# lukifer23/Matrix0

Measured on AMD Instinct MI355X. Metric: self-play games/sec at 800 sims/move, ResNet-24 53M; 1/2/4/8 MI355X, higher is better.
Workload: dtype f16

## Files before the change

matrix0_amd/csrc/attn_block.hip:

```cpp
#include "kernel_common.h"
#include "conv_epilogue.h"

typedef _Float16 half4v __attribute__((ext_vector_type(4)));
typedef float float4v __attribute__((ext_vector_type(4)));

namespace {
constexpr int AB_PIECE = 12288;
constexpr int AB_PIECES_PER_GROUP = 7;
constexpr int AB_GROUPS = 10;
constexpr int AB_X = 0;
constexpr int AB_QK = 81920;
constexpr int AB_VT = AB_QK + 16384;
constexpr int AB_VROW = 68;
constexpr int AB_RING = AB_VT + 4 * 16 * AB_VROW * 2;
constexpr int AB_PAR = AB_RING + 4 * AB_PIECE;
constexpr int AB_LDS = AB_PAR + 4 * 320 * 4;
}

__device__ __forceinline__ void ab_load64(half8& b0, half8& b1, half8& b2, half8& b3, const half8* p) {
    asm volatile("global_load_dwordx4 %0, %4, off\n\tglobal_load_dwordx4 %1, %4, off offset:16\n\t"
                 "global_load_dwordx4 %2, %4, off offset:32\n\tglobal_load_dwordx4 %3, %4, off offset:48"
                 : "=&v"(b0), "=&v"(b1), "=&v"(b2), "=&v"(b3) : "v"(p) : "memory");
}
template <int OFF>
__device__ __forceinline__ void ab_lds16(half8& d, uint32_t addr) {
    asm volatile("ds_read_b128 %0, %1 offset:%2" : "=v"(d) : "v"(addr), "n"(OFF) : "memory");
}
template <int N>
__device__ __forceinline__ void ab_lds_arrived(half8& f0, half8& f1, half8& f2, half8& f3, half8& f4, half8& f5) {
    static_assert(N == 0 || N == 5, "");
    if constexpr (N == 0) asm volatile("s_waitcnt lgkmcnt(0)" : "+v"(f0), "+v"(f1), "+v"(f2), "+v"(f3), "+v"(f4), "+v"(f5) :: "memory");
    else asm volatile("s_waitcnt lgkmcnt(5)" : "+v"(f0), "+v"(f1), "+v"(f2), "+v"(f3), "+v"(f4), "+v"(f5) :: "memory");
}
template <int CTRL>
__device__ __forceinline__ float ab_dpp(float v) {
    return __builtin_bit_cast(float, __builtin_amdgcn_update_dpp(0, __builtin_bit_cast(int, v), CTRL, 0xF, 0xF, true));
}
__device__ __forceinline__ float ab_row_sum(float v) {
    v += ab_dpp<0xB1>(v);
    v += ab_dpp<0x4E>(v);
    v += ab_dpp<0x141>(v);
    v += ab_dpp<0x140>(v);
    return v;
}

#ifndef AB_DBG
#define AB_DBG 0
#endif
#define AB_WAIT(n) asm volatile("s_waitcnt vmcnt(" #n ")" ::: "memory")
#if defined(AB_STAMP) || defined(AB_STAMP2) || defined(AB_STAMP3)
__device__ unsigned long long* g_ab_stamp;
#ifdef AB_STAMP
#define AB_ST(k) do { if (tid == 0) g_ab_stamp[(size_t)blockIdx.x * 16 + (k)] = __builtin_amdgcn_s_memtime(); } while (0)
#else
#define AB_ST(k) do {} while (0)
#endif
#else
#define AB_ST(k) do {} while (0)
#endif
#define AB_LGKM0() asm volatile("s_waitcnt lgkmcnt(0)" ::: "memory")
#ifdef AB_STAMP3
#define AB_T3(k) do { if (g == 5) ts[k] = __builtin_amdgcn_s_memtime(); } while (0)
#else
#define AB_T3(k) do {} while (0)
#endif
#ifdef AB_STAMP2
#define AB_TS(k) do { if (g == 5) ts[k] = __builtin_amdgcn_s_memtime(); } while (0)
#else
#define AB_TS(k) do {} while (0)
#endif

template <int ACT>
__global__ __launch_bounds__(512) void attn_block_kernel(AttnBlockArgs a) {
    extern __shared__ __attribute__((aligned(16))) char smem[];
    const int tid = threadIdx.x, lane = tid & 63;
    const int w = __builtin_amdgcn_readfirstlane(tid >> 6);
    const int l15 = lane & 15, lq = lane >> 4, r31 = lane & 31, half = lane >> 5;
    const int wm = w >> 1, wn = w & 1;
    const size_t b0 = (size_t)blockIdx.x * 2;
    const char* xg = reinterpret_cast<const char*>(a.x) + b0 * 64 * 640;

    AB_ST(0);
#pragma unroll
    for (int n = 0; n < 10; ++n) {
        const int idx = w * 10 + n;
        const int q = idx * 64 + lane;
        const int row = q / 40, pos = q - row * 40;
        const int src = (pos & ~7) | ((pos ^ (row >> 1)) & 7);
        glds16(xg + row * 640 + src * 16, smem + AB_X + idx * 1024);
    }
    const char* wsrc = reinterpret_cast<const char*>(a.wpack) + w * 1536 + lane * 16;
    char* const ring_w = smem + AB_RING + w * 1536;
    auto issue = [&](int t) __attribute__((always_inline)) {
        const char* s = wsrc + (size_t)t * AB_PIECE;
        char* d = ring_w + (t & 3) * AB_PIECE;
        glds16(s, d);
        if (lane < 32) glds16(s + 1024, d + 1024);
    };
    issue(0); issue(1); issue(2);
    if (tid < 320) {
        float* par = reinterpret_cast<float*>(smem + AB_PAR);
        par[tid] = a.ln_g[tid]; par[320 + tid] = a.ln_b[tid];
        par[640 + tid] = a.y2 ? a.gn2_gamma[tid] : 0.f; par[960 + tid] = a.y2 ? a.gn2_beta[tid] : 0.f;
    }

#if AB_DBG == 3
    AB_WAIT(0);
    __syncthreads();
    if (blockIdx.x == 0)
        for (int i = tid; i < 3 * AB_PIECE / 4; i += 512)
            reinterpret_cast<uint32_t*>(a.y)[i] = reinterpret_cast<const uint32_t*>(smem + AB_RING)[i];
    return;
#endif
    const int au = w >> 1, aboard = au >> 1, ahl = au & 1, aqt = w & 1;
    const int aq = aqt * 32 + r31;
    half2v visp[16];
    {
        const uint64_t m = a.mask[aq];
        static_for<0, 32>([&](auto i_) __attribute__((always_inline)) {
            constexpr int i = decltype(i_)::value;
            constexpr int kt = i >> 4, r = i & 15;
            const int key = kt * 32 + 8 * (r >> 2) + 4 * half + (r & 3);
            visp[i >> 1][i & 1] = (_Float16)(float)((m >> key) & 1);
        });
    }
    float wm_, wu_;
    if (a.mix > 0.f && a.mix < 1.f) { wm_ = 1.f - a.mix; wu_ = 1.f - (1.f - a.mix); }
    else if (a.mix >= 1.f) { wm_ = 1.f; wu_ = 0.f; }
    else { wm_ = 0.f; wu_ = 1.f; }
    const float isd = a.inv_sqrt_d * 1.44269504088896f;
    const float clampv = 50.f * 1.44269504088896f;

    const int xrow0 = 32 * wm + l15;
    const int xsw = (xrow0 >> 1) & 7;
    const int xe0 = ((lq ^ xsw) & 7) * 16, xe1 = (((4 + lq) ^ xsw) & 7) * 16;
    const uint32_t lds0 = (uint32_t)(uintptr_t)smem;
    const uint32_t xa[2] = {lds0 + AB_X + xrow0 * 640 + xe0, lds0 + AB_X + xrow0 * 640 + xe1};
    const int wsw = (l15 >> 1) & 7;
    const int wq0 = (3 * wn * 16 + l15) * 128 + ((lq ^ wsw) & 7) * 16;
    const int wq1 = (3 * wn * 16 + l15) * 128 + (((4 + lq) ^ wsw) & 7) * 16;
    const int wpo = l15 * 64 + ((lq ^ (4 - (l15 >> 2))) & 3) * 16;
    const uint32_t ring_a = lds0 + AB_RING;
    const uint32_t of_a = lds0 + AB_QK + (lq >> 1) * 4096 + (16 * w + l15) * 32 + ((lq & 1) ^ (l15 >> 3)) * 16;

    const float4v zero4 = {0.f, 0.f, 0.f, 0.f};
    const float16v zero16 = {0.f, 0.f, 0.f, 0.f, 0.f, 0.f, 0.f, 0.f, 0.f, 0.f, 0.f, 0.f, 0.f, 0.f, 0.f, 0.f};
    float4v oc[20];
    static_for<0, 20>([&](auto j_) __attribute__((always_inline)) { oc[decltype(j_)::value] = zero4; });

#if defined(AB_STAMP2) || defined(AB_STAMP3)
    unsigned long long ts[10] = {0, 0, 0, 0, 0, 0, 0, 0, 0, 0};
#endif
    half8 fs[2][5];
    half8 of;
    float4v qa[2][3];
    half8 bias8[4];
    auto sequence = [&](auto hp_, auto hq_, const int T, const int g) __attribute__((always_inline)) {
        constexpr bool HP = decltype(hp_)::value, HQ = decltype(hq_)::value;
        constexpr int NP = (HP ? 2 : 0) + (HQ ? 5 : 0), NU = 2 * NP;
        constexpr int BU = NU - 3;
        auto load = [&](auto u_) __attribute__((always_inline)) {
            constexpr int u = decltype(u_)::value, S = u & 1, i = u >> 1, kk = u & 1;
            const uint32_t slot = ring_a + (uint32_t)(((T + i) & 3) * AB_PIECE);
            if constexpr (HP && i < 2) {
                if constexpr (u == 0) ab_lds16<0>(of, of_a);
                const uint32_t pa = slot + wpo;
                static_for<0, 5>([&](auto jj_) __attribute__((always_inline)) {
                    constexpr int jj = decltype(jj_)::value;
                    ab_lds16<(5 * kk + jj) * 1024>(fs[S][jj], pa);
                });
            } else {
                constexpr int p = i - (HP ? 2 : 0);
                ab_lds16<128 * p>(fs[S][3], xa[kk]);
                ab_lds16<128 * p + 16 * 640>(fs[S][4], xa[kk]);
                const uint32_t wa = slot + (kk ? wq1 : wq0);
                static_for<0, 3>([&](auto j_) __attribute__((always_inline)) {
                    constexpr int j = decltype(j_)::value;
                    ab_lds16<j * 2048>(fs[S][j], wa);
                });
            }
        };
        auto arrived = [&](auto u_, auto n_) __attribute__((always_inline)) {
            constexpr int S = decltype(u_)::value & 1;
            ab_lds_arrived<decltype(n_)::value>(fs[S][0], fs[S][1], fs[S][2], fs[S][3], fs[S][4], of);
        };
        auto mma = [&](auto u_) __attribute__((always_inline)) {
            constexpr int u = decltype(u_)::value, S = u & 1, i = u >> 1, kk = u & 1;
            if constexpr (HP && i < 2) {
                static_for<0, 5>([&](auto jj_) __attribute__((always_inline)) {
                    constexpr int c = 10 * i + 5 * kk + decltype(jj_)::value;
                    oc[c] = __builtin_amdgcn_mfma_f32_16x16x32_f16(fs[S][decltype(jj_)::value], of, oc[c], 0, 0, 0);
                });
            } else {
                static_for<0, 3>([&](auto j_) __attribute__((always_inline)) {
                    constexpr int j = decltype(j_)::value;
                    qa[0][j] = __builtin_amdgcn_mfma_f32_16x16x32_f16(fs[S][j], fs[S][3], qa[0][j], 0, 0, 0);
                    qa[1][j] = __builtin_amdgcn_mfma_f32_16x16x32_f16(fs[S][j], fs[S][4], qa[1][j], 0, 0, 0);
                });
            }
        };
        if constexpr (HP && HQ) AB_TS(0);
        AB_LGKM0();
        AB_WAIT(4);
        __builtin_amdgcn_s_barrier();
        asm volatile("" ::: "memory");
        if constexpr (HP && HQ) AB_TS(1);
        load(std::integral_constant<int, 0>{});
        issue(T + 3);
        static_for<0, NU>([&](auto u_) __attribute__((always_inline)) {
            constexpr int u = decltype(u_)::value;
            if constexpr (u + 1 < NU) {
                if constexpr (u & 1) {
                    if constexpr (HP && HQ && u == 7) AB_T3(7);
                    arrived(u_, std::integral_constant<int, 0>{});
                    if constexpr (HP && HQ && u == 7) AB_T3(8);
                    AB_WAIT(4);
                    __builtin_amdgcn_s_barrier();
                    asm volatile("" ::: "memory");
                    if constexpr (HP && HQ && u == 5) AB_T3(0);
                    if constexpr (HP && HQ && u == 7) AB_T3(9);
                    if constexpr (HP && HQ && (u == 1 || u == 3 || u == 7 || u == 11)) { if (g == 5) AB_ST(u == 1 ? 12 : u == 3 ? 13 : u == 7 ? 14 : 15); }
                    if constexpr (HP && HQ) AB_TS(2 + (u >> 1));
                }
                load(std::integral_constant<int, u + 1>{});
                if constexpr (HP && HQ && u == 5) AB_T3(1);
                if constexpr (HP && HQ && u == 6) AB_T3(4);
                if constexpr (u & 1) issue(T + (u >> 1) + 4);
                else arrived(u_, std::integral_constant<int, 5>{});
                if constexpr (HP && HQ && u == 5) AB_T3(2);
                if constexpr (HP && HQ && u == 6) AB_T3(5);
            } else {
                arrived(u_, std::integral_constant<int, 0>{});
            }
            if constexpr (HQ && u == BU) {
                const half8* bp = reinterpret_cast<const half8*>(a.bias) + ((size_t)((2 * g + ahl) * 2 + aqt) * 64 + lane) * 4;
                ab_load64(bias8[0], bias8[1], bias8[2], bias8[3], bp);
            }
            mma(u_);
            __builtin_amdgcn_sched_barrier(0);
            if constexpr (HP && HQ && u == 5) AB_T3(3);
            if constexpr (HP && HQ && u == 6) AB_T3(6);
            if constexpr (HP && HQ && u == NU - 1) AB_TS(8);
        });
    };

    auto zero_qa = [&]() __attribute__((always_inline)) {
        static_for<0, 2>([&](auto i_) __attribute__((always_inline)) {
            static_for<0, 3>([&](auto j_) __attribute__((always_inline)) { qa[decltype(i_)::value][decltype(j_)::value] = zero4; });
        });
    };
    auto stage_and_attend = [&](const int g) __attribute__((always_inline)) {
        if (g == 5) AB_ST(5);
        static_for<0, 2>([&](auto i_) __attribute__((always_inline)) {
            static_for<0, 3>([&](auto j_) __attribute__((always_inline)) {
                constexpr int i = decltype(i_)::value, j = decltype(j_)::value;
                const int J = 3 * wn + j, type = J >> 1, hl = J & 1;
                const int token = 32 * wm + 16 * i + l15;
                const half4v h = {(_Float16)qa[i][j][0], (_Float16)qa[i][j][1], (_Float16)qa[i][j][2], (_Float16)qa[i][j][3]};
                if (type < 2) {
                    *reinterpret_cast<half4v*>(smem + AB_QK + type * 8192 + hl * 4096 + token * 32 + (((lq >> 1) ^ (l15 >> 3)) & 1) * 16 + (lq & 1) * 8) = h;
                } else {
                    const int unit = (token >> 6) * 2 + hl, sq = token & 63;
                    union { half2v h2; uint32_t u; } p01, p23;
                    p01.h2 = half2v{h[0], h[1]}; p23.h2 = half2v{h[2], h[3]};
                    const bool odd = (lane & 1) != 0;
                    const uint32_t own = odd ? p23.u : p01.u;
                    const uint32_t recv = (uint32_t)__builtin_amdgcn_update_dpp(0, (int)(odd ? p01.u : p23.u), 0xB1, 0xF, 0xF, true);
                    const uint32_t ta = odd ? recv : own, tb = odd ? own : recv;
                    const uint32_t w0 = __builtin_amdgcn_perm(tb, ta, 0x05040100u);
                    const uint32_t w1 = __builtin_amdgcn_perm(tb, ta, 0x07060302u);
                    uint32_t* vt = reinterpret_cast<uint32_t*>(reinterpret_cast<_Float16*>(smem + AB_VT) +
                                                               (unit * 16 + 4 * lq + (odd ? 2 : 0)) * AB_VROW + (sq & ~1));
                    vt[0] = w0; vt[AB_VROW / 2] = w1;
                }
            });
        });
        AB_LGKM0();
        __builtin_amdgcn_s_barrier();
        asm volatile("" ::: "memory");
        if (g == 5) AB_ST(6);
        AB_TS(9);
        if (AB_DBG != 2) {
            const char* Kb = smem + AB_QK + 8192 + ahl * 4096 + aboard * 64 * 32;
            const int hsw = 16 * (half ^ ((r31 >> 3) & 1));
            const half8 kf0 = *reinterpret_cast<const half8*>(Kb + r31 * 32 + hsw);
            const half8 kf1 = *reinterpret_cast<const half8*>(Kb + (32 + r31) * 32 + hsw);
            char* Qp = smem + AB_QK + ahl * 4096 + (aboard * 64 + aq) * 32 + hsw;
            const half8 qfr = *reinterpret_cast<const half8*>(Qp);
            half8 vf[2][2];
            {
                const _Float16* vrow = reinterpret_cast<const _Float16*>(smem + AB_VT) + (au * 16 + l15) * AB_VROW;
                static_for<0, 2>([&](auto kt_) __attribute__((always_inline)) {
                    static_for<0, 2>([&](auto jb_) __attribute__((always_inline)) {
                        constexpr int kt = decltype(kt_)::value, jb = decltype(jb_)::value;
                        const half4v lo = *reinterpret_cast<const half4v*>(vrow + kt * 32 + 16 * jb + 4 * half);
                        const half4v hi = *reinterpret_cast<const half4v*>(vrow + kt * 32 + 16 * jb + 8 + 4 * half);
                        vf[kt][jb] = half8{lo[0], lo[1], lo[2], lo[3], hi[0], hi[1], hi[2], hi[3]};
                    });
                });
            }
            float16v st[2];
            st[0] = __builtin_amdgcn_mfma_f32_32x32x16_f16(kf0, qfr, zero16, 0, 0, 0);
            st[1] = __builtin_amdgcn_mfma_f32_32x32x16_f16(kf1, qfr, zero16, 0, 0, 0);
            asm volatile("s_waitcnt vmcnt(0)" : "+v"(bias8[0]), "+v"(bias8[1]), "+v"(bias8[2]), "+v"(bias8[3]) :: "memory");
            float e[2][16];
            float su = 0.f, sm = 0.f;
            static_for<0, 2>([&](auto kt_) __attribute__((always_inline)) {
                static_for<0, 16>([&](auto r_) __attribute__((always_inline)) {
                    constexpr int kt = decltype(kt_)::value, r = decltype(r_)::value;
                    constexpr int bi = kt * 16 + r;
                    float d = st[kt][r] * isd + (float)bias8[bi >> 3][bi & 7];
                    d = __builtin_amdgcn_fmed3f(d, -clampv, clampv);
                    const float eu = __builtin_amdgcn_exp2f(d);
                    e[kt][r] = eu;
                    su += eu;
                    sm += eu * (float)visp[bi >> 1][bi & 1];
                });
            });
            su += __shfl_xor(su, 32);
            sm += __shfl_xor(sm, 32);
            const float cu = wu_ / su, cm = wm_ / sm;
            float16v oacc = zero16;
            static_for<0, 2>([&](auto kt_) __attribute__((always_inline)) {
                static_for<0, 2>([&](auto jb_) __attribute__((always_inline)) {
                    constexpr int kt = decltype(kt_)::value, jb = decltype(jb_)::value;
                    half8 pf;
                    static_for<0, 8>([&](auto u_) __attribute__((always_inline)) {
                        constexpr int u = decltype(u_)::value;
                        constexpr int r = 8 * jb + u, bi = kt * 16 + r;
                        const float vis = (float)visp[bi >> 1][bi & 1];
                        pf[u] = (_Float16)(e[kt][r] * (vis * cm + cu));
                    });
                    oacc = __builtin_amdgcn_mfma_f32_32x32x16_f16(vf[kt][jb], pf, oacc, 0, 0, 0);
                });
            });
            union { half2v h2[2]; uint32_t u[2]; } lo4, hi4, rcv;
            lo4.h2[0] = half2v{(_Float16)oacc[0], (_Float16)oacc[1]}; lo4.h2[1] = half2v{(_Float16)oacc[2], (_Float16)oacc[3]};
            hi4.h2[0] = half2v{(_Float16)oacc[4], (_Float16)oacc[5]}; hi4.h2[1] = half2v{(_Float16)oacc[6], (_Float16)oacc[7]};
            rcv.u[0] = __shfl_xor(half ? lo4.u[0] : hi4.u[0], 32);
            rcv.u[1] = __shfl_xor(half ? lo4.u[1] : hi4.u[1], 32);
            typedef uint32_t uint4v __attribute__((ext_vector_type(4)));
            uint4v ov;
            if (half == 0) ov = uint4v{lo4.u[0], lo4.u[1], rcv.u[0], rcv.u[1]};
            else ov = uint4v{rcv.u[0], rcv.u[1], hi4.u[0], hi4.u[1]};
            asm volatile("ds_write_b128 %0, %1" :: "v"((uint32_t)(uintptr_t)Qp), "v"(ov) : "memory");
        }
        if (g == 5) AB_ST(7);
    };

    if (AB_DBG != 1) {
        zero_qa();
        sequence(std::false_type{}, std::true_type{}, 0, 0);
#pragma unroll 1
        for (int g = 0; g < AB_GROUPS - 1; ++g) {
            stage_and_attend(g);
            if (g == 4) AB_ST(8);
            if (g == 5) AB_ST(11);
            zero_qa();
            sequence(std::true_type{}, std::true_type{}, 7 * g + 5, g + 1);
        }
        stage_and_attend(AB_GROUPS - 1);
        sequence(std::true_type{}, std::false_type{}, 7 * AB_GROUPS - 2, AB_GROUPS);
    }
    AB_ST(2);
#if defined(AB_STAMP2) || defined(AB_STAMP3)
    if (lane == 0 && (w & 3) == 0)
        for (int k = 0; k < 10; ++k) g_ab_stamp[((size_t)blockIdx.x * 2 + (w >> 2)) * 16 + k] = ts[k];
#endif
    AB_WAIT(0);
    __syncthreads();

    const int token = 16 * w + l15;
    const int tsw = (token >> 1) & 7;
    char* xrow = smem + AB_X + token * 640 + (lq & 1) * 8;
    float s1 = 0.f, s2 = 0.f;
    static_for<0, 20>([&](auto j_) __attribute__((always_inline)) {
        constexpr int j = decltype(j_)::value;
        const int chunk = 2 * j + (lq >> 1);
        const int pos = (chunk & ~7) | ((chunk ^ tsw) & 7);
        const half4v xv = *reinterpret_cast<const half4v*>(xrow + pos * 16);
        static_for<0, 4>([&](auto r_) __attribute__((always_inline)) {
            constexpr int r = decltype(r_)::value;
            const float v = oc[j][r] + (float)xv[r];
            oc[j][r] = v;
            s1 += v; s2 += v * v;
        });
    });
    s1 += __shfl_xor(s1, 16); s2 += __shfl_xor(s2, 16);
    s1 += __shfl_xor(s1, 32); s2 += __shfl_xor(s2, 32);
    const float cnt = (float)a.ln_count;
    const float mean = s1 / cnt;
    float var = s2 / cnt - mean * mean;
    var = var > 0.f ? var : 0.f;
    const float rstd = rsqrtf(var + 1e-5f);
    const float* par = reinterpret_cast<const float*>(smem + AB_PAR);
    float2* scr = reinterpret_cast<float2*>(smem + AB_RING);
    float2* tot = scr + 8 * 20 * 4;
    const float nmr = -mean * rstd;
    static_for<0, 20>([&](auto j_) __attribute__((always_inline)) {
        constexpr int j = decltype(j_)::value;
        const float4 gm = *reinterpret_cast<const float4*>(par + 16 * j + 4 * lq);
        const float4 bt = *reinterpret_cast<const float4*>(par + 320 + 16 * j + 4 * lq);
        const float gmv[4] = {gm.x, gm.y, gm.z, gm.w}, btv[4] = {bt.x, bt.y, bt.z, bt.w};
        float p1 = 0.f, p2 = 0.f;
        half4v h;
        static_for<0, 4>([&](auto r_) __attribute__((always_inline)) {
            constexpr int r = decltype(r_)::value;
            const float y = fmaf(fmaf(oc[j][r], rstd, nmr), gmv[r], btv[r]);
            p1 += y; p2 += y * y;
            h[r] = (_Float16)y;
        });
        const int chunk = 2 * j + (lq >> 1);
        const int pos = (chunk & ~7) | ((chunk ^ tsw) & 7);
        *reinterpret_cast<half4v*>(xrow + pos * 16) = h;
        p1 = ab_row_sum(p1); p2 = ab_row_sum(p2);
        if (l15 == 0) scr[(w * 20 + j) * 4 + lq] = make_float2(p1, p2);
    });
    auto flush = [&](_Float16* outp) __attribute__((always_inline)) {
        char* og = reinterpret_cast<char*>(outp) + (b0 * 64 + 16 * w) * 640;
#pragma unroll
        for (int n = 0; n < 10; ++n) {
            const int q = n * 64 + lane;
            const int rl = q / 40, pos = q - rl * 40;
            const int grow = 16 * w + rl;
            const int src = (pos & ~7) | ((pos ^ (grow >> 1)) & 7);
            const uint4 v = *reinterpret_cast<const uint4*>(smem + AB_X + grow * 640 + pos * 16);
            *reinterpret_cast<uint4*>(og + rl * 640 + src * 16) = v;
        }
    };
    AB_ST(3);
    flush(a.y);
    AB_ST(4);
    if (a.y2 == nullptr) return;
    __syncthreads();
    if (tid < 40) {
        const int bd = tid / 20, j = tid - bd * 20;
        float s = 0.f, ss = 0.f;
        for (int ww = 0; ww < 4; ++ww)
            for (int q = 0; q < 4; ++q) { const float2 v = scr[((bd * 4 + ww) * 20 + j) * 4 + q]; s += v.x; ss += v.y; }
        const float mu = s * (1.f / 1024.f);
        float vr = ss * (1.f / 1024.f) - mu * mu;
        vr = vr > 0.f ? vr : 0.f;
        tot[tid] = make_float2(mu, rsqrtf(vr + 1e-5f));
    }
    __syncthreads();
    {
        float* parw = reinterpret_cast<float*>(smem + AB_PAR);
        float scv[2] = {0.f, 0.f}, shv[2] = {0.f, 0.f};
        if (tid < 320) {
            const float g2 = parw[640 + tid], b2 = parw[960 + tid];
#pragma unroll
            for (int bd = 0; bd < 2; ++bd) {
                const float2 mr = tot[bd * 20 + (tid >> 4)];
                scv[bd] = g2 * mr.y; shv[bd] = b2 - mr.x * scv[bd];
            }
        }
        __syncthreads();
        if (tid < 320) { parw[tid] = scv[0]; parw[320 + tid] = shv[0]; parw[640 + tid] = scv[1]; parw[960 + tid] = shv[1]; }
        __syncthreads();
    }
    static_for<0, 20>([&](auto j_) __attribute__((always_inline)) {
        constexpr int j = decltype(j_)::value;
        const float4 gm = *reinterpret_cast<const float4*>(par + (w >> 2) * 640 + 16 * j + 4 * lq);
        const float4 bt = *reinterpret_cast<const float4*>(par + (w >> 2) * 640 + 320 + 16 * j + 4 * lq);
        const float gmv[4] = {gm.x, gm.y, gm.z, gm.w}, btv[4] = {bt.x, bt.y, bt.z, bt.w};
        const int chunk = 2 * j + (lq >> 1);
        const int pos = (chunk & ~7) | ((chunk ^ tsw) & 7);
        half4v h = *reinterpret_cast<const half4v*>(xrow + pos * 16);
        static_for<0, 4>([&](auto r_) __attribute__((always_inline)) {
            constexpr int r = decltype(r_)::value;
            h[r] = (_Float16)act_fast<ACT>((float)h[r] * gmv[r] + btv[r]);
        });
        *reinterpret_cast<half4v*>(xrow + pos * 16) = h;
    });
    AB_ST(9);
    flush(a.y2);
    AB_ST(10);
}

hipError_t launch_attn_block(const AttnBlockArgs& a, hipStream_t st) {
    if (a.B <= 0 || a.B % 2 != 0 || a.ln_count <= 0 || a.ln_count > 320) return hipErrorInvalidValue;
    if (a.y2 != nullptr && a.act != ACT_SILU && a.act != ACT_RELU) return hipErrorInvalidValue;
    static DeviceOnce once;
    hipError_t e = once.run([] {
        hipError_t r = hipFuncSetAttribute(reinterpret_cast<const void*>(&attn_block_kernel<ACT_SILU>),
                                           hipFuncAttributeMaxDynamicSharedMemorySize, AB_LDS);
        if (r != hipSuccess) return r;
        return hipFuncSetAttribute(reinterpret_cast<const void*>(&attn_block_kernel<ACT_RELU>),
                                   hipFuncAttributeMaxDynamicSharedMemorySize, AB_LDS);
    });
    if (e != hipSuccess) return e;
    const dim3 grid((unsigned)(a.B / 2));
    if (a.act == ACT_RELU) hipLaunchKernelGGL(attn_block_kernel<ACT_RELU>, grid, dim3(512), AB_LDS, st, a);
    else hipLaunchKernelGGL(attn_block_kernel<ACT_SILU>, grid, dim3(512), AB_LDS, st, a);
    return hipGetLastError();
}

size_t attn_block_pack_bytes() { return (size_t)(AB_GROUPS * AB_PIECES_PER_GROUP + 3) * AB_PIECE; }
```

matrix0_amd/csrc/net_kernels.h:

```cpp
#pragma once
#include <hip/hip_runtime.h>
#include <stdint.h>

enum { ACT_NONE = 0, ACT_RELU = 1, ACT_SILU = 2, ACT_LEAKY = 3, ACT_SIGMOID = 4, ACT_TANH = 5 };

constexpr int TAIL_SE_HMAX = 96;

struct GemmArgs {
    const _Float16* in;
    const _Float16* w;
    void* out;
    const float* gn_gamma;
    const float* gn_beta;
    const float* bias;
    const _Float16* mul;
    float* out_stats;
    int Mrows;
    int Mvalid;
    int Cin;
    int N;
    int Npad;
    int ldo;
    int epi_act;
    int out_f32;
    float out_scale;
    int ksplit;
    int w_pp;
    const _Float16* res;
    const float* pre_gamma;
    const float* pre_beta;
    _Float16* y2;
    const float* se_w1;
    const float* se_b1;
    const float* se_w2;
    const float* se_b2;
    int se_hidden;
    const void* se_wf;
    const float* posenc;
    void* out2;
    int ldo2;
    int nsplit;
};

struct EwArgs {
    const _Float16* t;
    const float* t_stats;
    const float* gn_gamma;
    const float* gn_beta;
    const float* gate;
    const _Float16* res;
    const float* posenc;
    const float* ln_g;
    const float* ln_b;
    int ln_count;
    _Float16* y;
    float* out_stats;
    _Float16* y2;
    const float* gn2_gamma;
    const float* gn2_beta;
    int C;
    int act;
};

struct SeGateArgs {
    const float* t_stats;
    const float* w1;
    const float* b1;
    const float* w2;
    const float* b2;
    float* gate;
    int B, C, hidden, act;
};

struct AttnArgs {
    const _Float16* qkv;
    const float* rel_bias;
    const uint64_t* mask;
    _Float16* o;
    int B, H, C;
    float mix;
    float inv_sqrt_d;
};

struct AttnBlockArgs {
    const _Float16* x;
    const void* wpack;
    const _Float16* bias;
    const uint64_t* mask;
    const float* ln_g;
    const float* ln_b;
    const float* gn2_gamma;
    const float* gn2_beta;
    _Float16* y;
    _Float16* y2;
    int B;
    int ln_count;
    int act;
    float mix;
    float inv_sqrt_d;
};
hipError_t launch_attn_block(const AttnBlockArgs& a, hipStream_t st);
hipError_t launch_splitk_reduce(const float* part, int splits, int M, int N, const float* bias, int act, _Float16* out,
                                hipStream_t st);
size_t attn_block_pack_bytes();

hipError_t launch_conv_gemm(const GemmArgs& a, int taps, hipStream_t st);
int conv_gemm_tile_n(int Cin, int Npad);
int conv_gemm_kc(int Cin, int Npad);
hipError_t launch_ew_board(const EwArgs& a, int boards, hipStream_t st);
hipError_t launch_se_gate(const SeGateArgs& a, hipStream_t st);
hipError_t launch_attn_core(const AttnArgs& a, hipStream_t st);
hipError_t launch_planes_to_nhwc(const float* x, void* y, int B, int P, hipStream_t st);
hipError_t launch_nhwc_to_nchw_f32(const void* x, float* y, int B, int ld, int n, int ctot, int coff, hipStream_t st);
```

Before: 1.167.

## Make attention block kernel persistent and prefetch next board pair during epilogue

The attention block kernel becomes persistent: the grid is capped at the CU count and each workgroup loops over board pairs. While the LayerNorm/GroupNorm epilogue of the current pair runs, most of the next pair's input is prefetched into spare LDS staging areas, then copied into the X buffer. The intent is to hide input load latency and launch/tail costs when B/2 exceeds the CU count. It adds LDS-to-LDS copies, extra barriers and more LDS use, and it gives up parallelism when there are fewer pairs than CUs.

```diff
diff --git a/matrix0_amd/csrc/attn_block.hip b/matrix0_amd/csrc/attn_block.hip
--- a/matrix0_amd/csrc/attn_block.hip
+++ b/matrix0_amd/csrc/attn_block.hip
@@ -1,5 +1,7 @@
 #include "kernel_common.h"
 #include "conv_epilogue.h"
+#include <algorithm>
+#include <atomic>
 
 typedef _Float16 half4v __attribute__((ext_vector_type(4)));
 typedef float float4v __attribute__((ext_vector_type(4)));
@@ -14,7 +16,19 @@
 constexpr int AB_VROW = 68;
 constexpr int AB_RING = AB_VT + 4 * 16 * AB_VROW * 2;
 constexpr int AB_PAR = AB_RING + 4 * AB_PIECE;
-constexpr int AB_LDS = AB_PAR + 4 * 320 * 4;
+constexpr int AB_SC1 = AB_PAR + 4 * 320 * 4;
+constexpr int AB_LDS = AB_SC1 + 2 * 320 * 4;
+constexpr int AB_SCR = AB_RING;
+constexpr int AB_SCR_BYTES = (8 * 20 * 4 + 2 * 20) * 8;
+constexpr int AB_SC0 = AB_PAR - 2 * 320 * 4;
+constexpr int AB_UNIT = 1024;
+constexpr int AB_STG_UNITS = 8;
+constexpr int AB_STG_A = AB_QK;
+constexpr int AB_STG_A_WAVES = 3;
+constexpr int AB_STG_B = AB_SCR + AB_SCR_BYTES;
+static_assert(AB_STG_A + AB_STG_A_WAVES * AB_STG_UNITS * AB_UNIT <= AB_RING, "staging area A runs into the GroupNorm partials");
+static_assert(AB_STG_B + (8 - AB_STG_A_WAVES) * AB_STG_UNITS * AB_UNIT <= AB_SC0, "staging area B runs into the scale / shift table");
+static_assert(AB_STG_B % 16 == 0 && AB_LDS <= 160 * 1024, "");
 }
 
 __device__ __forceinline__ void ab_load64(half8& b0, half8& b1, half8& b2, half8& b3, const half8* p) {
@@ -22,9 +36,24 @@
                  "global_load_dwordx4 %2, %4, off offset:32\n\tglobal_load_dwordx4 %3, %4, off offset:48"
                  : "=&v"(b0), "=&v"(b1), "=&v"(b2), "=&v"(b3) : "v"(p) : "memory");
 }
+__device__ __forceinline__ void ab_glds16_untracked(const void* gsrc, uint32_t lds_wave_base) {
+    uint32_t m0_kept;
+    asm volatile("s_mov_b32 %0, m0\n\ts_mov_b32 m0, %1\n\ts_nop 0\n\tglobal_load_lds_dwordx4 %2, off\n\ts_mov_b32 m0, %0"
+                 : "=&s"(m0_kept) : "s"(lds_wave_base), "v"(gsrc) : "memory");
+}
+__device__ __forceinline__ void ab_glds16_lower_half(const void* gsrc, uint32_t lds_wave_base) {
+    uint32_t m0_kept, exec_hi_kept;
+    asm volatile("s_mov_b32 %0, m0\n\ts_mov_b32 %1, exec_hi\n\ts_mov_b32 exec_hi, 0\n\ts_mov_b32 m0, %2\n\ts_nop 0\n\t"
+                 "global_load_lds_dwordx4 %3, off\n\ts_mov_b32 exec_hi, %1\n\ts_mov_b32 m0, %0"
+                 : "=&s"(m0_kept), "=&s"(exec_hi_kept) : "s"(lds_wave_base), "v"(gsrc) : "memory");
+}
 template <int OFF>
 __device__ __forceinline__ void ab_lds16(half8& d, uint32_t addr) {
     asm volatile("ds_read_b128 %0, %1 offset:%2" : "=v"(d) : "v"(addr), "n"(OFF) : "memory");
+}
+template <int OFF>
+__device__ __forceinline__ void ab_lds_write16(uint32_t addr, const half8& v) {
+    asm volatile("ds_write_b128 %0, %1 offset:%2" :: "v"(addr), "v"(v), "n"(OFF) : "memory");
 }
 template <int N>
 __device__ __forceinline__ void ab_lds_arrived(half8& f0, half8& f1, half8& f2, half8& f3, half8& f4, half8& f5) {
@@ -51,14 +80,18 @@
 #if defined(AB_STAMP) || defined(AB_STAMP2) || defined(AB_STAMP3)
 __device__ unsigned long long* g_ab_stamp;
 #ifdef AB_STAMP
-#define AB_ST(k) do { if (tid == 0) g_ab_stamp[(size_t)blockIdx.x * 16 + (k)] = __builtin_amdgcn_s_memtime(); } while (0)
+#define AB_ST(k) AB_STP(pair, k)
+#define AB_STP(p, k) do { if (tid == 0) g_ab_stamp[(size_t)(p) * 32 + (k)] = __builtin_amdgcn_s_memtime(); } while (0)
 #else
 #define AB_ST(k) do {} while (0)
+#define AB_STP(p, k) do {} while (0)
 #endif
 #else
 #define AB_ST(k) do {} while (0)
+#define AB_STP(p, k) do {} while (0)
 #endif
 #define AB_LGKM0() asm volatile("s_waitcnt lgkmcnt(0)" ::: "memory")
+#define AB_BAR() do { AB_LGKM0(); __builtin_amdgcn_s_barrier(); asm volatile("" ::: "memory"); } while (0)
 #ifdef AB_STAMP3
 #define AB_T3(k) do { if (g == 5) ts[k] = __builtin_amdgcn_s_memtime(); } while (0)
 #else
@@ -77,17 +110,20 @@
     const int w = __builtin_amdgcn_readfirstlane(tid >> 6);
     const int l15 = lane & 15, lq = lane >> 4, r31 = lane & 31, half = lane >> 5;
     const int wm = w >> 1, wn = w & 1;
-    const size_t b0 = (size_t)blockIdx.x * 2;
-    const char* xg = reinterpret_cast<const char*>(a.x) + b0 * 64 * 640;
+    const int npairs = a.B >> 1;
+    int pair = blockIdx.x;
+    auto unit_src = [&](int n, int lane) __attribute__((always_inline)) {
+        const int q = (w * 10 + n) * 64 + lane;
+        const int row = q / 40, pos = q - row * 40;
+        return row * 640 + ((pos & ~7) | ((pos ^ (row >> 1)) & 7)) * 16;
+    };
+    auto pair_rows = [&](int p) __attribute__((always_inline)) { return reinterpret_cast<const char*>(a.x) + (size_t)p * (128 * 640); };
 
     AB_ST(0);
+    {
+        const char* xg = pair_rows(pair);
 #pragma unroll
-    for (int n = 0; n < 10; ++n) {
-        const int idx = w * 10 + n;
-        const int q = idx * 64 + lane;
-        const int row = q / 40, pos = q - row * 40;
-        const int src = (pos & ~7) | ((pos ^ (row >> 1)) & 7);
-        glds16(xg + row * 640 + src * 16, smem + AB_X + idx * 1024);
+        for (int n = 0; n < 10; ++n) glds16(xg + unit_src(n, lane), smem + AB_X + (w * 10 + n) * AB_UNIT);
     }
     const char* wsrc = reinterpret_cast<const char*>(a.wpack) + w * 1536 + lane * 16;
     char* const ring_w = smem + AB_RING + w * 1536;
@@ -95,7 +131,7 @@
         const char* s = wsrc + (size_t)t * AB_PIECE;
         char* d = ring_w + (t & 3) * AB_PIECE;
         glds16(s, d);
-        if (lane < 32) glds16(s + 1024, d + 1024);
+        ab_glds16_lower_half(s + 1024, (uint32_t)(uintptr_t)d + 1024);
     };
     issue(0); issue(1); issue(2);
     if (tid < 320) {
@@ -142,11 +178,12 @@
     const int wpo = l15 * 64 + ((lq ^ (4 - (l15 >> 2))) & 3) * 16;
     const uint32_t ring_a = lds0 + AB_RING;
     const uint32_t of_a = lds0 + AB_QK + (lq >> 1) * 4096 + (16 * w + l15) * 32 + ((lq & 1) ^ (l15 >> 3)) * 16;
+    const uint32_t stg_w = lds0 + (w < AB_STG_A_WAVES ? AB_STG_A + w * AB_STG_UNITS * AB_UNIT
+                                                      : AB_STG_B + (w - AB_STG_A_WAVES) * AB_STG_UNITS * AB_UNIT);
 
     const float4v zero4 = {0.f, 0.f, 0.f, 0.f};
     const float16v zero16 = {0.f, 0.f, 0.f, 0.f, 0.f, 0.f, 0.f, 0.f, 0.f, 0.f, 0.f, 0.f, 0.f, 0.f, 0.f, 0.f};
     float4v oc[20];
-    static_for<0, 20>([&](auto j_) __attribute__((always_inline)) { oc[decltype(j_)::value] = zero4; });
 
 #if defined(AB_STAMP2) || defined(AB_STAMP3)
     unsigned long long ts[10] = {0, 0, 0, 0, 0, 0, 0, 0, 0, 0};
@@ -205,6 +242,7 @@
         __builtin_amdgcn_s_barrier();
         asm volatile("" ::: "memory");
         if constexpr (HP && HQ) AB_TS(1);
+        if constexpr (!HP) AB_ST(18);
         load(std::integral_constant<int, 0>{});
         issue(T + 3);
         static_for<0, NU>([&](auto u_) __attribute__((always_inline)) {
@@ -348,149 +386,216 @@
         if (g == 5) AB_ST(7);
     };
 
-    if (AB_DBG != 1) {
-        zero_qa();
-        sequence(std::false_type{}, std::true_type{}, 0, 0);
 #pragma unroll 1
-        for (int g = 0; g < AB_GROUPS - 1; ++g) {
-            stage_and_attend(g);
-            if (g == 4) AB_ST(8);
-            if (g == 5) AB_ST(11);
+    for (;;) {
+        const size_t b0 = (size_t)pair * 2;
+        const int next = pair + (int)gridDim.x;
+        const bool has_next = next < npairs;
+        asm volatile("" : "+v"(wsrc));
+        static_for<0, 20>([&](auto j_) __attribute__((always_inline)) { oc[decltype(j_)::value] = zero4; });
+        if (AB_DBG != 1) {
             zero_qa();
-            sequence(std::true_type{}, std::true_type{}, 7 * g + 5, g + 1);
-        }
-        stage_and_attend(AB_GROUPS - 1);
-        sequence(std::true_type{}, std::false_type{}, 7 * AB_GROUPS - 2, AB_GROUPS);
-    }
-    AB_ST(2);
+            sequence(std::false_type{}, std::true_type{}, 0, 0);
+            AB_ST(1);
+#pragma unroll 1
+            for (int g = 0; g < AB_GROUPS - 1; ++g) {
+                stage_and_attend(g);
+                if (g == 4) AB_ST(8);
+                if (g == 5) AB_ST(11);
+                zero_qa();
+                sequence(std::true_type{}, std::true_type{}, 7 * g + 5, g + 1);
+            }
+            stage_and_attend(AB_GROUPS - 1);
+            sequence(std::true_type{}, std::false_type{}, 7 * AB_GROUPS - 2, AB_GROUPS);
+        }
+        AB_ST(2);
 #if defined(AB_STAMP2) || defined(AB_STAMP3)
-    if (lane == 0 && (w & 3) == 0)
-        for (int k = 0; k < 10; ++k) g_ab_stamp[((size_t)blockIdx.x * 2 + (w >> 2)) * 16 + k] = ts[k];
-#endif
-    AB_WAIT(0);
-    __syncthreads();
-
-    const int token = 16 * w + l15;
-    const int tsw = (token >> 1) & 7;
-    char* xrow = smem + AB_X + token * 640 + (lq & 1) * 8;
-    float s1 = 0.f, s2 = 0.f;
-    static_for<0, 20>([&](auto j_) __attribute__((always_inline)) {
-        constexpr int j = decltype(j_)::value;
-        const int chunk = 2 * j + (lq >> 1);
-        const int pos = (chunk & ~7) | ((chunk ^ tsw) & 7);
-        const half4v xv = *reinterpret_cast<const half4v*>(xrow + pos * 16);
-        static_for<0, 4>([&](auto r_) __attribute__((always_inline)) {
-            constexpr int r = decltype(r_)::value;
-            const float v = oc[j][r] + (float)xv[r];
-            oc[j][r] = v;
-            s1 += v; s2 += v * v;
+        if (lane == 0 && (w & 3) == 0)
+            for (int k = 0; k < 10; ++k) g_ab_stamp[((size_t)pair * 2 + (w >> 2)) * 16 + k] = ts[k];
+#endif
+        __builtin_amdgcn_s_waitcnt(0);
+        __builtin_amdgcn_s_barrier();
+        asm volatile("" ::: "memory");
+        {
+        int tid_o = threadIdx.x;
+        asm volatile("" : "+v"(tid_o));
+        const int tid = tid_o, lane = tid & 63, l15 = lane & 15, lq = lane >> 4;
+        if (has_next) {
+            const char* xn = pair_rows(next);
+            static_for<0, AB_STG_UNITS>([&](auto n_) __attribute__((always_inline)) {
+                constexpr int n = decltype(n_)::value;
+                ab_glds16_untracked(xn + unit_src(n, lane), stg_w + n * AB_UNIT);
+            });
+        }
+        AB_ST(16);
+
+        const int token = 16 * w + l15;
+        const int tsw = (token >> 1) & 7;
+        char* xrow = smem + AB_X + token * 640 + (lq & 1) * 8;
+        float s1 = 0.f, s2 = 0.f;
+        static_for<0, 20>([&](auto j_) __attribute__((always_inline)) {
+            constexpr int j = decltype(j_)::value;
+            const int chunk = 2 * j + (lq >> 1);
+            const int pos = (chunk & ~7) | ((chunk ^ tsw) & 7);
+            const half4v xv = *reinterpret_cast<const half4v*>(xrow + pos * 16);
+            static_for<0, 4>([&](auto r_) __attribute__((always_inline)) {
+                constexpr int r = decltype(r_)::value;
+                const float v = oc[j][r] + (float)xv[r];
+                oc[j][r] = v;
+                s1 += v; s2 += v * v;
+            });
         });
-    });
-    s1 += __shfl_xor(s1, 16); s2 += __shfl_xor(s2, 16);
-    s1 += __shfl_xor(s1, 32); s2 += __shfl_xor(s2, 32);
-    const float cnt = (float)a.ln_count;
-    const float mean = s1 / cnt;
-    float var = s2 / cnt - mean * mean;
-    var = var > 0.f ? var : 0.f;
-    const float rstd = rsqrtf(var + 1e-5f);
-    const float* par = reinterpret_cast<const float*>(smem + AB_PAR);
-    float2* scr = reinterpret_cast<float2*>(smem + AB_RING);
-    float2* tot = scr + 8 * 20 * 4;
-    const float nmr = -mean * rstd;
-    static_for<0, 20>([&](auto j_) __attribute__((always_inline)) {
-        constexpr int j = decltype(j_)::value;
-        const float4 gm = *reinterpret_cast<const float4*>(par + 16 * j + 4 * lq);
-        const float4 bt = *reinterpret_cast<const float4*>(par + 320 + 16 * j + 4 * lq);
-        const float gmv[4] = {gm.x, gm.y, gm.z, gm.w}, btv[4] = {bt.x, bt.y, bt.z, bt.w};
-        float p1 = 0.f, p2 = 0.f;
-        half4v h;
-        static_for<0, 4>([&](auto r_) __attribute__((always_inline)) {
-            constexpr int r = decltype(r_)::value;
-            const float y = fmaf(fmaf(oc[j][r], rstd, nmr), gmv[r], btv[r]);
-            p1 += y; p2 += y * y;
-            h[r] = (_Float16)y;
+        s1 += __shfl_xor(s1, 16); s2 += __shfl_xor(s2, 16);
+        s1 += __shfl_xor(s1, 32); s2 += __shfl_xor(s2, 32);
+        const float cnt = (float)a.ln_count;
+        const float mean = s1 / cnt;
+        float var = s2 / cnt - mean * mean;
+        var = var > 0.f ? var : 0.f;
+        const float rstd = rsqrtf(var + 1e-5f);
+        const float* par = reinterpret_cast<const float*>(smem + AB_PAR);
+        float2* scr = reinterpret_cast<float2*>(smem + AB_SCR);
+        float2* tot = scr + 8 * 20 * 4;
+        const float nmr = -mean * rstd;
+        static_for<0, 20>([&](auto j_) __attribute__((always_inline)) {
+            constexpr int j = decltype(j_)::value;
+            const float4 gm = *reinterpret_cast<const float4*>(par + 16 * j + 4 * lq);
+            const float4 bt = *reinterpret_cast<const float4*>(par + 320 + 16 * j + 4 * lq);
+            const float gmv[4] = {gm.x, gm.y, gm.z, gm.w}, btv[4] = {bt.x, bt.y, bt.z, bt.w};
+            float p1 = 0.f, p2 = 0.f;
+            half4v h;
+            static_for<0, 4>([&](auto r_) __attribute__((always_inline)) {
+                constexpr int r = decltype(r_)::value;
+                const float y = fmaf(fmaf(oc[j][r], rstd, nmr), gmv[r], btv[r]);
+                p1 += y; p2 += y * y;
+                h[r] = (_Float16)y;
+            });
+            const int chunk = 2 * j + (lq >> 1);
+            const int pos = (chunk & ~7) | ((chunk ^ tsw) & 7);
+            *reinterpret_cast<half4v*>(xrow + pos * 16) = h;
+            p1 = ab_row_sum(p1); p2 = ab_row_sum(p2);
+            if (l15 == 0) scr[(w * 20 + j) * 4 + lq] = make_float2(p1, p2);
         });
-        const int chunk = 2 * j + (lq >> 1);
-        const int pos = (chunk & ~7) | ((chunk ^ tsw) & 7);
-        *reinterpret_cast<half4v*>(xrow + pos * 16) = h;
-        p1 = ab_row_sum(p1); p2 = ab_row_sum(p2);
-        if (l15 == 0) scr[(w * 20 + j) * 4 + lq] = make_float2(p1, p2);
-    });
-    auto flush = [&](_Float16* outp) __attribute__((always_inline)) {
-        char* og = reinterpret_cast<char*>(outp) + (b0 * 64 + 16 * w) * 640;
+        auto flush = [&](_Float16* outp) __attribute__((always_inline)) {
+            char* og = reinterpret_cast<char*>(outp) + (b0 * 64 + 16 * w) * 640;
 #pragma unroll
-        for (int n = 0; n < 10; ++n) {
-            const int q = n * 64 + lane;
-            const int rl = q / 40, pos = q - rl * 40;
-            const int grow = 16 * w + rl;
-            const int src = (pos & ~7) | ((pos ^ (grow >> 1)) & 7);
-            const uint4 v = *reinterpret_cast<const uint4*>(smem + AB_X + grow * 640 + pos * 16);
-            *reinterpret_cast<uint4*>(og + rl * 640 + src * 16) = v;
-        }
-    };
-    AB_ST(3);
-    flush(a.y);
-    AB_ST(4);
-    if (a.y2 == nullptr) return;
-    __syncthreads();
-    if (tid < 40) {
-        const int bd = tid / 20, j = tid - bd * 20;
-        float s = 0.f, ss = 0.f;
-        for (int ww = 0; ww < 4; ++ww)
-            for (int q = 0; q < 4; ++q) { const float2 v = scr[((bd * 4 + ww) * 20 + j) * 4 + q]; s += v.x; ss += v.y; }
-        const float mu = s * (1.f / 1024.f);
-        float vr = ss * (1.f / 1024.f) - mu * mu;
-        vr = vr > 0.f ? vr : 0.f;
-        tot[tid] = make_float2(mu, rsqrtf(vr + 1e-5f));
-    }
-    __syncthreads();
-    {
-        float* parw = reinterpret_cast<float*>(smem + AB_PAR);
-        float scv[2] = {0.f, 0.f}, shv[2] = {0.f, 0.f};
+            for (int n = 0; n < 10; ++n) {
+                const int q = n * 64 + lane;
+                const int rl = q / 40, pos = q - rl * 40;
+                const int grow = 16 * w + rl;
+                const int src = (pos & ~7) | ((pos ^ (grow >> 1)) & 7);
+                const uint4 v = *reinterpret_cast<const uint4*>(smem + AB_X + grow * 640 + pos * 16);
+                *reinterpret_cast<uint4*>(og + rl * 640 + src * 16) = v;
+            }
+        };
+        AB_ST(3);
+        flush(a.y);
+        AB_ST(4);
+        if (a.y2 != nullptr) {
+        AB_BAR();
+        if (tid < 40) {
+            const int bd = tid / 20, j = tid - bd * 20;
+            float s = 0.f, ss = 0.f;
+            for (int ww = 0; ww < 4; ++ww)
+                for (int q = 0; q < 4; ++q) { const float2 v = scr[((bd * 4 + ww) * 20 + j) * 4 + q]; s += v.x; ss += v.y; }
+            const float mu = s * (1.f / 1024.f);
+            float vr = ss * (1.f / 1024.f) - mu * mu;
+            vr = vr > 0.f ? vr : 0.f;
+            tot[tid] = make_float2(mu, rsqrtf(vr + 1e-5f));
+        }
+        AB_BAR();
         if (tid < 320) {
-            const float g2 = parw[640 + tid], b2 = parw[960 + tid];
+            const float g2 = par[640 + tid], b2 = par[960 + tid];
 #pragma unroll
             for (int bd = 0; bd < 2; ++bd) {
                 const float2 mr = tot[bd * 20 + (tid >> 4)];
-                scv[bd] = g2 * mr.y; shv[bd] = b2 - mr.x * scv[bd];
-            }
-        }
-        __syncthreads();
-        if (tid < 320) { parw[tid] = scv[0]; parw[320 + tid] = shv[0]; parw[640 + tid] = scv[1]; parw[960 + tid] = shv[1]; }
-        __syncthreads();
+                const float sc = g2 * mr.y, sh = b2 - mr.x * sc;
+                float* t = reinterpret_cast<float*>(smem + (bd ? AB_SC1 : AB_SC0));
+                t[tid] = sc; t[320 + tid] = sh;
+            }
+        }
+        AB_BAR();
+        const float* scsh = reinterpret_cast<const float*>(smem + ((w >> 2) ? AB_SC1 : AB_SC0));
+        static_for<0, 20>([&](auto j_) __attribute__((always_inline)) {
+            constexpr int j = decltype(j_)::value;
+            const float4 gm = *reinterpret_cast<const float4*>(scsh + 16 * j + 4 * lq);
+            const float4 bt = *reinterpret_cast<const float4*>(scsh + 320 + 16 * j + 4 * lq);
+            const float gmv[4] = {gm.x, gm.y, gm.z, gm.w}, btv[4] = {bt.x, bt.y, bt.z, bt.w};
+            const int chunk = 2 * j + (lq >> 1);
+            const int pos = (chunk & ~7) | ((chunk ^ tsw) & 7);
+            half4v h = *reinterpret_cast<const half4v*>(xrow + pos * 16);
+            static_for<0, 4>([&](auto r_) __attribute__((always_inline)) {
+                constexpr int r = decltype(r_)::value;
+                h[r] = (_Float16)act_fast<ACT>((float)h[r] * gmv[r] + btv[r]);
+            });
+            *reinterpret_cast<half4v*>(xrow + pos * 16) = h;
+        });
+        AB_ST(9);
+        flush(a.y2);
+        AB_ST(10);
+        }
+        if (!has_next) break;
+        AB_STP(next, 0);
+        AB_WAIT(0);
+        {
+            half8 t[AB_STG_UNITS];
+            static_for<0, AB_STG_UNITS>([&](auto n_) __attribute__((always_inline)) {
+                constexpr int n = decltype(n_)::value;
+                ab_lds16<n * AB_UNIT>(t[n], stg_w + lane * 16);
+            });
+            static_assert(AB_STG_UNITS == 8, "");
+            asm volatile("s_waitcnt lgkmcnt(0)" : "+v"(t[0]), "+v"(t[1]), "+v"(t[2]), "+v"(t[3]), "+v"(t[4]), "+v"(t[5]), "+v"(t[6]), "+v"(t[7]) :: "memory");
+            static_for<0, AB_STG_UNITS>([&](auto n_) __attribute__((always_inline)) {
+                constexpr int n = decltype(n_)::value;
+                ab_lds_write16<n * AB_UNIT>(lds0 + AB_X + w * 10 * AB_UNIT + lane * 16, t[n]);
+            });
+        }
+        {
+            const char* xn = pair_rows(next);
+#pragma unroll
+            for (int n = AB_STG_UNITS; n < 10; ++n) glds16(xn + unit_src(n, lane), smem + AB_X + (w * 10 + n) * AB_UNIT);
+        }
+        AB_BAR();
+        AB_STP(next, 17);
+        }
+        issue(0); issue(1); issue(2);
+        pair = next;
     }
-    static_for<0, 20>([&](auto j_) __attribute__((always_inline)) {
-        constexpr int j = decltype(j_)::value;
-        const float4 gm = *reinterpret_cast<const float4*>(par + (w >> 2) * 640 + 16 * j + 4 * lq);
-        const float4 bt = *reinterpret_cast<const float4*>(par + (w >> 2) * 640 + 320 + 16 * j + 4 * lq);
-        const float gmv[4] = {gm.x, gm.y, gm.z, gm.w}, btv[4] = {bt.x, bt.y, bt.z, bt.w};
-        const int chunk = 2 * j + (lq >> 1);
-        const int pos = (chunk & ~7) | ((chunk ^ tsw) & 7);
-        half4v h = *reinterpret_cast<const half4v*>(xrow + pos * 16);
-        static_for<0, 4>([&](auto r_) __attribute__((always_inline)) {
-            constexpr int r = decltype(r_)::value;
-            h[r] = (_Float16)act_fast<ACT>((float)h[r] * gmv[r] + btv[r]);
-        });
-        *reinterpret_cast<half4v*>(xrow + pos * 16) = h;
+}
+
+static hipError_t ab_configure(int* cus) {
+    static DeviceOnce once;
+    static std::atomic<int> known[32];
+    int d = 0, fresh = 0;
+    if (hipGetDevice(&d) != hipSuccess) return hipErrorInvalidDevice;
+    const hipError_t e = once.run([&] {
+        hipError_t r = hipFuncSetAttribute(reinterpret_cast<const void*>(&attn_block_kernel<ACT_SILU>),
+                                           hipFuncAttributeMaxDynamicSharedMemorySize, AB_LDS);
+        if (r != hipSuccess) return r;
+        r = hipFuncSetAttribute(reinterpret_cast<const void*>(&attn_block_kernel<ACT_RELU>),
+                                hipFuncAttributeMaxDynamicSharedMemorySize, AB_LDS);
+        if (r != hipSuccess) return r;
+        r = hipDeviceGetAttribute(&fresh, hipDeviceAttributeMultiprocessorCount, d);
+        if (r != hipSuccess) return r;
+        if (fresh <= 0) return hipErrorInvalidDevice;
+        if ((unsigned)d < 32u) known[d].store(fresh, std::memory_order_relaxed);
+        return hipSuccess;
     });
-    AB_ST(9);
-    flush(a.y2);
-    AB_ST(10);
+    if (e != hipSuccess) return e;
+    *cus = fresh > 0 ? fresh : known[d].load(std::memory_order_relaxed);
+    return hipSuccess;
+}
+int attn_block_workgroups(int B) {
+    int cus = 0;
+    return ab_configure(&cus) == hipSuccess ? std::min(B / 2, cus) : -1;
 }
 
 hipError_t launch_attn_block(const AttnBlockArgs& a, hipStream_t st) {
     if (a.B <= 0 || a.B % 2 != 0 || a.ln_count <= 0 || a.ln_count > 320) return hipErrorInvalidValue;
     if (a.y2 != nullptr && a.act != ACT_SILU && a.act != ACT_RELU) return hipErrorInvalidValue;
-    static DeviceOnce once;
-    hipError_t e = once.run([] {
-        hipError_t r = hipFuncSetAttribute(reinterpret_cast<const void*>(&attn_block_kernel<ACT_SILU>),
-                                           hipFuncAttributeMaxDynamicSharedMemorySize, AB_LDS);
-        if (r != hipSuccess) return r;
-        return hipFuncSetAttribute(reinterpret_cast<const void*>(&attn_block_kernel<ACT_RELU>),
-                                   hipFuncAttributeMaxDynamicSharedMemorySize, AB_LDS);
-    });
+    int cus = 0;
+    const hipError_t e = ab_configure(&cus);
     if (e != hipSuccess) return e;
-    const dim3 grid((unsigned)(a.B / 2));
+    const dim3 grid((unsigned)std::min(a.B / 2, cus));
     if (a.act == ACT_RELU) hipLaunchKernelGGL(attn_block_kernel<ACT_RELU>, grid, dim3(512), AB_LDS, st, a);
     else hipLaunchKernelGGL(attn_block_kernel<ACT_SILU>, grid, dim3(512), AB_LDS, st, a);
     return hipGetLastError();
diff --git a/matrix0_amd/csrc/net_kernels.h b/matrix0_amd/csrc/net_kernels.h
--- a/matrix0_amd/csrc/net_kernels.h
+++ b/matrix0_amd/csrc/net_kernels.h
@@ -103,6 +103,7 @@
 hipError_t launch_splitk_reduce(const float* part, int splits, int M, int N, const float* bias, int act, _Float16* out,
                                 hipStream_t st);
 size_t attn_block_pack_bytes();
+int attn_block_workgroups(int B);
 
 hipError_t launch_conv_gemm(const GemmArgs& a, int taps, hipStream_t st);
 int conv_gemm_tile_n(int Cin, int Npad);
```

Result: faster. 1.182, median of 6 (+1.3%).
